# speechbrain/speechbrain

Measured on NVIDIA H100. Metric: audio-sec/sec (RTFx) Conformer-L ASR, batch=32x10s@16kHz, higher is better.
Workload: dtype fp16 operands, fp32 accumulate/residual/softmax

## Files before the change

### speechbrain_b200/csrc/common.cuh

```cuda
#pragma once
#include <cuda.h>
#include <cuda_fp16.h>
#include <cuda_runtime.h>
#include <stdint.h>

#define SBK_OK 0
#define SBK_ERR_CUDA -1
#define SBK_ERR_ARG -2
#define SBK_ERR_UNSUPPORTED -3
#define SBK_ERR_NOMEM -4

namespace sbk {

void set_error(const char* fmt, ...);

#define SBK_CUDA_CHECK(expr)                                                              \
    do {                                                                                  \
        cudaError_t _e = (expr);                                                          \
        if (_e != cudaSuccess) {                                                          \
            sbk::set_error("%s:%d: %s -> %s", __FILE__, __LINE__, #expr, cudaGetErrorString(_e)); \
            return SBK_ERR_CUDA;                                                          \
        }                                                                                 \
    } while (0)

// ... 20 lines not shown
__device__ __forceinline__ void pdl_wait() { asm volatile("griddepcontrol.wait;" ::: "memory"); }

template <typename... KArgs, typename... Args>
inline cudaError_t launch_pdl(void (*kern)(KArgs...), dim3 grid, dim3 block, size_t smem, cudaStream_t st, bool pdl,
                              Args... args) {
    cudaLaunchConfig_t cfg = {};
    cfg.gridDim = grid;
    cfg.blockDim = block;
    cfg.dynamicSmemBytes = smem;
    cfg.stream = st;
    cudaLaunchAttribute attr[1];
    attr[0].id = cudaLaunchAttributeProgrammaticStreamSerialization;
    attr[0].val.programmaticStreamSerializationAllowed = 1;
    cfg.attrs = attr;
    cfg.numAttrs = pdl ? 1 : 0;
    return cudaLaunchKernelEx(&cfg, kern, args...);
}

__device__ __forceinline__ float warp_sum(float v) {
#pragma unroll
    for (int o = 16; o > 0; o >>= 1) v += __shfl_xor_sync(0xffffffffu, v, o);
    return v;
}
__device__ __forceinline__ float warp_max(float v) {
#pragma unroll
    for (int o = 16; o > 0; o >>= 1) v = fmaxf(v, __shfl_xor_sync(0xffffffffu, v, o));
    return v;
}

__device__ __forceinline__ uint32_t smem_u32(const void* p) {
    return static_cast<uint32_t>(__cvta_generic_to_shared(p));
}

__device__ __forceinline__ void mbar_init(uint64_t* bar, uint32_t count) {
    asm volatile("mbarrier.init.shared::cta.b64 [%0], %1;" ::"r"(smem_u32(bar)), "r"(count));
}
__device__ __forceinline__ void mbar_fence_init() {
    asm volatile("fence.mbarrier_init.release.cluster;" ::: "memory");
}
__device__ __forceinline__ void mbar_arrive_expect_tx(uint64_t* bar, uint32_t bytes) {
    asm volatile("mbarrier.arrive.expect_tx.shared::cta.b64 _, [%0], %1;" ::"r"(smem_u32(bar)), "r"(bytes)
                 : "memory");
}
__device__ __forceinline__ void mbar_arrive(uint64_t* bar) {
    asm volatile("mbarrier.arrive.shared::cta.b64 _, [%0];" ::"r"(smem_u32(bar)) : "memory");
}
__device__ __forceinline__ bool mbar_try_wait(uint64_t* bar, uint32_t parity) {
    uint32_t ok;
    asm volatile(
        "{\n\t.reg .pred p;\n\t"
        "mbarrier.try_wait.parity.shared::cta.b64 p, [%1], %2;\n\t"
        "selp.u32 %0, 1, 0, p;\n\t}"
        : "=r"(ok)
        : "r"(smem_u32(bar)), "r"(parity)
        : "memory");
    return ok != 0;
}
__device__ __forceinline__ void mbar_wait(uint64_t* bar, uint32_t parity) {
    while (!mbar_try_wait(bar, parity)) {
    }
}

__device__ __forceinline__ void tma_prefetch_desc(const CUtensorMap* m) {
    asm volatile("prefetch.tensormap [%0];" ::"l"(reinterpret_cast<uint64_t>(m)) : "memory");
}
__device__ __forceinline__ void tma_load_2d(void* smem_dst, const CUtensorMap* m, uint64_t* bar, int c0, int c1) {
    asm volatile(
        "cp.async.bulk.tensor.2d.shared::cluster.global.mbarrier::complete_tx::bytes [%0], [%1, {%3, %4}], [%2];"
        ::"r"(smem_u32(smem_dst)), "l"(reinterpret_cast<uint64_t>(m)), "r"(smem_u32(bar)), "r"(c0), "r"(c1)
        : "memory");
}
__device__ __forceinline__ void tma_load_4d(void* smem_dst, const CUtensorMap* m, uint64_t* bar, int c0, int c1, int c2, int c3) {
    asm volatile(
        "cp.async.bulk.tensor.4d.shared::cluster.global.mbarrier::complete_tx::bytes [%0], [%1, {%3, %4, %5, %6}], [%2];"
        ::"r"(smem_u32(smem_dst)), "l"(reinterpret_cast<uint64_t>(m)), "r"(smem_u32(bar)), "r"(c0), "r"(c1), "r"(c2), "r"(c3)
        : "memory");
}
__device__ __forceinline__ void bulk_load_1d(void* smem_dst, const void* gsrc, uint32_t bytes, uint64_t* bar) {
    asm volatile(
        "cp.async.bulk.shared::cluster.global.mbarrier::complete_tx::bytes [%0], [%1], %2, [%3];"
        ::"r"(smem_u32(smem_dst)), "l"(reinterpret_cast<uint64_t>(gsrc)), "r"(bytes), "r"(smem_u32(bar))
        : "memory");
}

__device__ __forceinline__ void wgmma_fence() { asm volatile("wgmma.fence.sync.aligned;" ::: "memory"); }
__device__ __forceinline__ void wgmma_commit() { asm volatile("wgmma.commit_group.sync.aligned;" ::: "memory"); }
template <int N>
__device__ __forceinline__ void wgmma_wait() { asm volatile("wgmma.wait_group.sync.aligned %0;" ::"n"(N) : "memory"); }

__device__ __forceinline__ uint64_t make_kmajor_sw128_desc(uint32_t smem_addr) {
    uint64_t d = 0;
    d |= static_cast<uint64_t>((smem_addr & 0x3FFFFu) >> 4);
    d |= static_cast<uint64_t>(1) << 16;
    d |= static_cast<uint64_t>(1024 >> 4) << 32;
    d |= static_cast<uint64_t>(1) << 62;
    return d;
}

template <int N>
__device__ __forceinline__ void wgmma_f16(float (&d)[N / 2], uint64_t desc_a, uint64_t desc_b, uint32_t accumulate);
template <>
__device__ __forceinline__ void wgmma_f16<32>(float (&d)[16], uint64_t desc_a, uint64_t desc_b, uint32_t accumulate) {
    asm volatile(
        "{\n\t.reg .pred p;\n\tsetp.ne.b32 p, %18, 0;\n\t"
        "wgmma.mma_async.sync.aligned.m64n32k16.f32.f16.f16 "
        "{%0, %1, %2, %3, %4, %5, %6, %7, %8, %9, %10, %11, %12, %13, %14, %15}, "
        "%16, %17, p, 1, 1, 0, 0;\n\t}"
        : "+f"(d[0]), "+f"(d[1]), "+f"(d[2]), "+f"(d[3]), "+f"(d[4]), "+f"(d[5]), "+f"(d[6]), "+f"(d[7]),
          "+f"(d[8]), "+f"(d[9]), "+f"(d[10]), "+f"(d[11]), "+f"(d[12]), "+f"(d[13]), "+f"(d[14]), "+f"(d[15])
        : "l"(desc_a), "l"(desc_b), "r"(accumulate)
        : "memory");
}
template <>
__device__ __forceinline__ void wgmma_f16<64>(float (&d)[32], uint64_t desc_a, uint64_t desc_b, uint32_t accumulate) {
    asm volatile(
        "{\n\t.reg .pred p;\n\tsetp.ne.b32 p, %34, 0;\n\t"
        "wgmma.mma_async.sync.aligned.m64n64k16.f32.f16.f16 "
        "{%0, %1, %2, %3, %4, %5, %6, %7, %8, %9, %10, %11, %12, %13, %14, %15, "
        "%16, %17, %18, %19, %20, %21, %22, %23, %24, %25, %26, %27, %28, %29, %30, %31}, "
        "%32, %33, p, 1, 1, 0, 0;\n\t}"
        : "+f"(d[0]), "+f"(d[1]), "+f"(d[2]), "+f"(d[3]), "+f"(d[4]), "+f"(d[5]), "+f"(d[6]), "+f"(d[7]),
          "+f"(d[8]), "+f"(d[9]), "+f"(d[10]), "+f"(d[11]), "+f"(d[12]), "+f"(d[13]), "+f"(d[14]), "+f"(d[15]),
          "+f"(d[16]), "+f"(d[17]), "+f"(d[18]), "+f"(d[19]), "+f"(d[20]), "+f"(d[21]), "+f"(d[22]), "+f"(d[23]),
          "+f"(d[24]), "+f"(d[25]), "+f"(d[26]), "+f"(d[27]), "+f"(d[28]), "+f"(d[29]), "+f"(d[30]), "+f"(d[31])
        : "l"(desc_a), "l"(desc_b), "r"(accumulate)
        : "memory");
}
template <>
__device__ __forceinline__ void wgmma_f16<128>(float (&d)[64], uint64_t desc_a, uint64_t desc_b, uint32_t accumulate) {
    asm volatile(
        "{\n\t.reg .pred p;\n\tsetp.ne.b32 p, %66, 0;\n\t"
        "wgmma.mma_async.sync.aligned.m64n128k16.f32.f16.f16 "
        "{%0, %1, %2, %3, %4, %5, %6, %7, %8, %9, %10, %11, %12, %13, %14, %15, "
        "%16, %17, %18, %19, %20, %21, %22, %23, %24, %25, %26, %27, %28, %29, %30, %31, "
        "%32, %33, %34, %35, %36, %37, %38, %39, %40, %41, %42, %43, %44, %45, %46, %47, "
        "%48, %49, %50, %51, %52, %53, %54, %55, %56, %57, %58, %59, %60, %61, %62, %63}, "
        "%64, %65, p, 1, 1, 0, 0;\n\t}"
        : "+f"(d[0]), "+f"(d[1]), "+f"(d[2]), "+f"(d[3]), "+f"(d[4]), "+f"(d[5]), "+f"(d[6]), "+f"(d[7]),
          "+f"(d[8]), "+f"(d[9]), "+f"(d[10]), "+f"(d[11]), "+f"(d[12]), "+f"(d[13]), "+f"(d[14]), "+f"(d[15]),
          "+f"(d[16]), "+f"(d[17]), "+f"(d[18]), "+f"(d[19]), "+f"(d[20]), "+f"(d[21]), "+f"(d[22]), "+f"(d[23]),
          "+f"(d[24]), "+f"(d[25]), "+f"(d[26]), "+f"(d[27]), "+f"(d[28]), "+f"(d[29]), "+f"(d[30]), "+f"(d[31]),
          "+f"(d[32]), "+f"(d[33]), "+f"(d[34]), "+f"(d[35]), "+f"(d[36]), "+f"(d[37]), "+f"(d[38]), "+f"(d[39]),
          "+f"(d[40]), "+f"(d[41]), "+f"(d[42]), "+f"(d[43]), "+f"(d[44]), "+f"(d[45]), "+f"(d[46]), "+f"(d[47]),
          "+f"(d[48]), "+f"(d[49]), "+f"(d[50]), "+f"(d[51]), "+f"(d[52]), "+f"(d[53]), "+f"(d[54]), "+f"(d[55]),
          "+f"(d[56]), "+f"(d[57]), "+f"(d[58]), "+f"(d[59]), "+f"(d[60]), "+f"(d[61]), "+f"(d[62]), "+f"(d[63])
        : "l"(desc_a), "l"(desc_b), "r"(accumulate)
        : "memory");
}

template <>
__device__ __forceinline__ void wgmma_f16<256>(float (&d)[128], uint64_t desc_a, uint64_t desc_b, uint32_t accumulate) {
    asm volatile(
        "{\n\t.reg .pred p;\n\tsetp.ne.b32 p, %130, 0;\n\t"
        "wgmma.mma_async.sync.aligned.m64n256k16.f32.f16.f16 "
        "{"
        "%0, %1, %2, %3, %4, %5, %6, %7, %8, %9, %10, %11, %12, %13, %14, %15, "
        "%16, %17, %18, %19, %20, %21, %22, %23, %24, %25, %26, %27, %28, %29, %30, %31, "
        "%32, %33, %34, %35, %36, %37, %38, %39, %40, %41, %42, %43, %44, %45, %46, %47, "
        "%48, %49, %50, %51, %52, %53, %54, %55, %56, %57, %58, %59, %60, %61, %62, %63, "
        "%64, %65, %66, %67, %68, %69, %70, %71, %72, %73, %74, %75, %76, %77, %78, %79, "
        "%80, %81, %82, %83, %84, %85, %86, %87, %88, %89, %90, %91, %92, %93, %94, %95, "
        "%96, %97, %98, %99, %100, %101, %102, %103, %104, %105, %106, %107, %108, %109, %110, %111, "
        "%112, %113, %114, %115, %116, %117, %118, %119, %120, %121, %122, %123, %124, %125, %126, %127}, "
        "%128, %129, p, 1, 1, 0, 0;\n\t}"
        :
          "+f"(d[0]), "+f"(d[1]), "+f"(d[2]), "+f"(d[3]), "+f"(d[4]), "+f"(d[5]), "+f"(d[6]), "+f"(d[7]),
          "+f"(d[8]), "+f"(d[9]), "+f"(d[10]), "+f"(d[11]), "+f"(d[12]), "+f"(d[13]), "+f"(d[14]), "+f"(d[15]),
          "+f"(d[16]), "+f"(d[17]), "+f"(d[18]), "+f"(d[19]), "+f"(d[20]), "+f"(d[21]), "+f"(d[22]), "+f"(d[23]),
          "+f"(d[24]), "+f"(d[25]), "+f"(d[26]), "+f"(d[27]), "+f"(d[28]), "+f"(d[29]), "+f"(d[30]), "+f"(d[31]),
          "+f"(d[32]), "+f"(d[33]), "+f"(d[34]), "+f"(d[35]), "+f"(d[36]), "+f"(d[37]), "+f"(d[38]), "+f"(d[39]),
          "+f"(d[40]), "+f"(d[41]), "+f"(d[42]), "+f"(d[43]), "+f"(d[44]), "+f"(d[45]), "+f"(d[46]), "+f"(d[47]),
          "+f"(d[48]), "+f"(d[49]), "+f"(d[50]), "+f"(d[51]), "+f"(d[52]), "+f"(d[53]), "+f"(d[54]), "+f"(d[55]),
          "+f"(d[56]), "+f"(d[57]), "+f"(d[58]), "+f"(d[59]), "+f"(d[60]), "+f"(d[61]), "+f"(d[62]), "+f"(d[63]),
          "+f"(d[64]), "+f"(d[65]), "+f"(d[66]), "+f"(d[67]), "+f"(d[68]), "+f"(d[69]), "+f"(d[70]), "+f"(d[71]),
          "+f"(d[72]), "+f"(d[73]), "+f"(d[74]), "+f"(d[75]), "+f"(d[76]), "+f"(d[77]), "+f"(d[78]), "+f"(d[79]),
          "+f"(d[80]), "+f"(d[81]), "+f"(d[82]), "+f"(d[83]), "+f"(d[84]), "+f"(d[85]), "+f"(d[86]), "+f"(d[87]),
          "+f"(d[88]), "+f"(d[89]), "+f"(d[90]), "+f"(d[91]), "+f"(d[92]), "+f"(d[93]), "+f"(d[94]), "+f"(d[95]),
          "+f"(d[96]), "+f"(d[97]), "+f"(d[98]), "+f"(d[99]), "+f"(d[100]), "+f"(d[101]), "+f"(d[102]), "+f"(d[103]),
          "+f"(d[104]), "+f"(d[105]), "+f"(d[106]), "+f"(d[107]), "+f"(d[108]), "+f"(d[109]), "+f"(d[110]), "+f"(d[111]),
          "+f"(d[112]), "+f"(d[113]), "+f"(d[114]), "+f"(d[115]), "+f"(d[116]), "+f"(d[117]), "+f"(d[118]), "+f"(d[119]),
          "+f"(d[120]), "+f"(d[121]), "+f"(d[122]), "+f"(d[123]), "+f"(d[124]), "+f"(d[125]), "+f"(d[126]), "+f"(d[127])
        : "l"(desc_a), "l"(desc_b), "r"(accumulate)
        : "memory");
}

__device__ __forceinline__ __half2 floats2half2_sat(float lo, float hi) {
    uint32_t r;
    asm("cvt.rn.satfinite.f16x2.f32 %0, %1, %2;" : "=r"(r) : "f"(hi), "f"(lo));
    return *reinterpret_cast<__half2*>(&r);
}
__device__ __forceinline__ __half float2half_sat(float x) {
    const __half2 h = floats2half2_sat(x, 0.0f);
    return __low2half(h);
}

__device__ __forceinline__ float rcp_approx(float x) {
    float y;
    asm("rcp.approx.ftz.f32 %0, %1;" : "=f"(y) : "f"(x));
    return y;
}
__device__ __forceinline__ float exp_ftz(float x) {
    float y;
    asm("ex2.approx.ftz.f32 %0, %1;" : "=f"(y) : "f"(x * 1.4426950408889634f));
    return y;
}
__device__ __forceinline__ float sigmoid_f(float x) { return rcp_approx(1.0f + exp_ftz(-x)); }
__device__ __forceinline__ float tanh_approx(float x) {
    float y;
    asm("tanh.approx.f32 %0, %1;" : "=f"(y) : "f"(x));
    return y;
}
__device__ __forceinline__ float sigmoid_fast(float x) { return fmaf(0.5f, tanh_approx(0.5f * x), 0.5f); }
__device__ __forceinline__ float silu_fast(float x) {
    const float h = 0.5f * x;
    return fmaf(h, tanh_approx(h), h);
}
__device__ __forceinline__ void sts128(uint32_t addr, uint4 v) {
    asm volatile("st.shared.v4.b32 [%0], {%1, %2, %3, %4};" ::"r"(addr), "r"(v.x), "r"(v.y), "r"(v.z), "r"(v.w) : "memory");
}
__device__ __forceinline__ uint4 lds128(uint32_t addr) {
    uint4 v;
    asm volatile("ld.shared.v4.b32 {%0, %1, %2, %3}, [%4];" : "=r"(v.x), "=r"(v.y), "=r"(v.z), "=r"(v.w) : "r"(addr) : "memory");
    return v;
}
__device__ __forceinline__ uint4 f4_as_u4(float4 f) {
    return make_uint4(__float_as_uint(f.x), __float_as_uint(f.y), __float_as_uint(f.z), __float_as_uint(f.w));
}
__device__ __forceinline__ float4 u4_as_f4(uint4 u) {
    return make_float4(__uint_as_float(u.x), __uint_as_float(u.y), __uint_as_float(u.z), __uint_as_float(u.w));
}
__device__ __forceinline__ float silu_f(float x) { return x * sigmoid_f(x); }
__device__ __forceinline__ float gelu_erf_f(float x) { return 0.5f * x * (1.0f + erff(x * 0.70710678118654752f)); }

__device__ __forceinline__ int float_to_ordered(float f) {
    int i = __float_as_int(f);
    return i >= 0 ? i : i ^ 0x7FFFFFFF;
}
__device__ __forceinline__ float ordered_to_float(int i) { return __int_as_float(i >= 0 ? i : i ^ 0x7FFFFFFF); }

int make_tmap_2d_f16(CUtensorMap* out, const void* base, uint64_t rows, uint64_t cols, uint64_t row_stride_elems,
                     uint32_t box_rows, uint32_t box_cols);

}
```

### speechbrain_b200/csrc/gemm_tc2.cu

```cuda
#include <stdio.h>
#include <stdlib.h>

#include "common.cuh"
#include "sbk_internal.h"

namespace sbk {

constexpr int PP_BM = 128, PP_BK = 64;
constexpr int PP_THREADS = 384;
constexpr int PP_GROUP_M = 8;
constexpr int PP_A_BYTES = PP_BM * PP_BK * 2;
constexpr int PP_STG_WARP_BYTES = 16 * 160;
constexpr int PP_BAR_TURN = 2;
constexpr int PP_CONSUMER_REGS = 232, PP_PRODUCER_REGS = 40;
static_assert(128 * PP_PRODUCER_REGS + 256 * PP_CONSUMER_REGS <= 65536, "register file");

template <int BN>
struct PpCfg {
    static constexpr bool PINGPONG = BN == 128;
    static constexpr int STAGES = BN == 128 ? 6 : 4;
    static constexpr int STAGE_BYTES = PP_A_BYTES + BN * PP_BK * 2;
    static constexpr int BAR_OFFSET = STAGES * STAGE_BYTES;
    static constexpr int STG_OFFSET = BAR_OFFSET + 128;
    static constexpr int BIAS_OFFSET = STG_OFFSET + 8 * PP_STG_WARP_BYTES;
    static constexpr int SMEM = BIAS_OFFSET + 8 * BN * 4 + 1024;
    static_assert(STAGE_BYTES % 1024 == 0, "128B-swizzled stages must stay 1 KB aligned");
    static_assert(2 * STAGES * 8 <= 128, "mbarriers overflow their slot");
    static_assert(SMEM <= 227 * 1024, "shared memory");
};

template <int MODE>
__host__ __device__ constexpr int pp_stg_pitch() {
    return (MODE == EPI_F32 || MODE == EPI_RESID) ? 160 : MODE == EPI_ROPE ? 144 : 80;
}

__device__ __forceinline__ void named_bar_sync(int id, int n) { asm volatile("bar.sync %0, %1;" ::"r"(id), "r"(n) : "memory"); }
__device__ __forceinline__ void named_bar_arrive(int id, int n) { asm volatile("bar.arrive %0, %1;" ::"r"(id), "r"(n) : "memory"); }
template <int R>
__device__ __forceinline__ void setmaxnreg_inc() { asm volatile("setmaxnreg.inc.sync.aligned.u32 %0;" ::"n"(R)); }
template <int R>
__device__ __forceinline__ void setmaxnreg_dec() { asm volatile("setmaxnreg.dec.sync.aligned.u32 %0;" ::"n"(R)); }
__device__ __forceinline__ void sts32(uint32_t addr, uint32_t v) { asm volatile("st.shared.b32 [%0], %1;" ::"r"(addr), "r"(v) : "memory"); }
__device__ __forceinline__ void sts64(uint32_t addr, float x, float y) {
    asm volatile("st.shared.v2.f32 [%0], {%1, %2};" ::"r"(addr), "f"(x), "f"(y) : "memory");
}
__device__ __forceinline__ float2 lds64(uint32_t addr) {
    float2 v;
    asm volatile("ld.shared.v2.f32 {%0, %1}, [%2];" : "=f"(v.x), "=f"(v.y) : "r"(addr) : "memory");
    return v;
}
__device__ __forceinline__ uint32_t half2_bits(float lo, float hi) {
    const __half2 h = floats2half2_sat(lo, hi);
    return *reinterpret_cast<const uint32_t*>(&h);
}

template <int BN>
__device__ __forceinline__ void pp_tile_coords(int t, int tiles_m, int tiles_n, int& m0, int& n0) {
    const int per_group = PP_GROUP_M * tiles_n;
    const int grp = t / per_group, first_m = grp * PP_GROUP_M;
    const int rows = min(PP_GROUP_M, tiles_m - first_m);
    const int r = t - grp * per_group;
    m0 = (first_m + r % rows) * PP_BM;
    n0 = (r / rows) * BN;
}


template <int MODE>
__device__ __forceinline__ void pp_row_alpha(const GemmEpilogue& e, float (&alpha)[2], int row_base, int M, int lane) {
#pragma unroll
    for (int i = 0; i < 2; ++i) {
        const int row = row_base + (lane >> 2) + 8 * i;
        alpha[i] = e.alpha;
        if (MODE == EPI_RESID && e.row_lens != nullptr && row < M) {
            const int b = row / e.T, t = row - b * e.T;
            if (t >= __ldg(e.row_lens + b)) alpha[i] = 0.0f;
        }
    }
}

__device__ __forceinline__ void pp_resid_prefetch(const GemmEpilogue& e, float4 (&res)[4], int row_base, int col0, int M,
                                                  int lane) {
    const int seg = lane & 7, rsub = lane >> 3;
#pragma unroll
    for (int i = 0; i < 4; ++i) {
        const int row = row_base + i * 4 + rsub;
        res[i] = row < M ? __ldcg(reinterpret_cast<const float4*>(e.resid + static_cast<size_t>(row) * e.ldo + col0 + seg * 4))
                         : make_float4(0.f, 0.f, 0.f, 0.f);
    }
}
__device__ __forceinline__ void pp_rope_prefetch(const GemmEpilogue& e, float4 (&rc)[2], float4 (&rs)[2], int row_base,
                                                 int col0, int lane) {
    const int dh = e.head_dim;
    const int within = col0 % (3 * dh);
    const int sect = within / dh;
    if (sect < 2) {
        const int p = ((within - sect * dh) >> 1) + (lane & 3) * 4;
#pragma unroll
        for (int i = 0; i < 2; ++i) {
            const int t = (row_base + i * 8 + (lane >> 2)) % e.T;
            rc[i] = __ldg(reinterpret_cast<const float4*>(e.rope_cos + static_cast<size_t>(t) * (dh >> 1) + p));
            rs[i] = __ldg(reinterpret_cast<const float4*>(e.rope_sin + static_cast<size_t>(t) * (dh >> 1) + p));
        }
    }
}
template <int MODE>
__device__ __forceinline__ void pp_prefetch(const GemmEpilogue& e, float4 (&res)[4], float4 (&rc)[2], float4 (&rs)[2],
                                            int row_base, int col0, int M, int lane) {
    if constexpr (MODE == EPI_RESID) pp_resid_prefetch(e, res, row_base, col0, M, lane);
    if constexpr (MODE == EPI_ROPE) pp_rope_prefetch(e, rc, rs, row_base, col0, lane);
// ... 59 lines not shown
            if (row < M) {
                float4 val = u4_as_f4(lds128(stg + r * P + seg * 16));
                if constexpr (MODE == EPI_RESID) {
                    val.x += res[i].x; val.y += res[i].y; val.z += res[i].z; val.w += res[i].w;
                }
                *reinterpret_cast<float4*>(outp + static_cast<size_t>(row) * e.ldo + col0 + seg * 4) = val;
            }
        }
    } else if constexpr (MODE == EPI_ROPE) {
        const int seg = lane & 3, rsub = lane >> 2;
        const int dh = e.head_dim;
        const int sect = (col0 % (3 * dh)) / dh;
        const float sc = sect == 0 ? e.alpha : 1.0f;
        __half* outp = reinterpret_cast<__half*>(e.out);
#pragma unroll
        for (int i = 0; i < 2; ++i) {
            const int r = i * 8 + rsub;
            const int row = row_base + r;
            float4 x0 = u4_as_f4(lds128(stg + r * P + seg * 32));
            float4 x1 = u4_as_f4(lds128(stg + r * P + seg * 32 + 16));
            if (sect < 2) {
                const float4 c = rc[i], s4 = rs[i];
                const float a0 = (x0.x * c.x - x0.y * s4.x) * sc, a1 = (x0.y * c.x + x0.x * s4.x) * sc;
                const float a2 = (x0.z * c.y - x0.w * s4.y) * sc, a3 = (x0.w * c.y + x0.z * s4.y) * sc;
                const float b0 = (x1.x * c.z - x1.y * s4.z) * sc, b1 = (x1.y * c.z + x1.x * s4.z) * sc;
                const float b2 = (x1.z * c.w - x1.w * s4.w) * sc, b3 = (x1.w * c.w + x1.z * s4.w) * sc;
                x0 = make_float4(a0, a1, a2, a3);
                x1 = make_float4(b0, b1, b2, b3);
            }
            if (row < M)
                *reinterpret_cast<uint4*>(outp + static_cast<size_t>(row) * e.ldo + col0 + seg * 8) =
                    make_uint4(half2_bits(x0.x, x0.y), half2_bits(x0.z, x0.w), half2_bits(x1.x, x1.y), half2_bits(x1.z, x1.w));
        }
    } else {
        const int seg = lane & 3, rsub = lane >> 2;
        if (MODE == EPI_F16 && e.kv_heads > 0) {
            const int d = e.kv_heads * 64;
            const int layer = col0 / (2 * d), within = col0 - layer * 2 * d;
            const int part = within / d, cc = within - part * d, head = cc >> 6, dcol = cc & 63;
            __half* pbase = reinterpret_cast<__half*>(e.out) + static_cast<size_t>(layer) * e.kv_layer_stride +
                            static_cast<size_t>(part) * e.kv_part_stride;
#pragma unroll
            for (int i = 0; i < 2; ++i) {
                const int r = i * 8 + rsub;
                const int row = row_base + r;
                if (row < M) {
                    const int b = row / e.T, t = row - b * e.T;
                    __half* dst = pbase + ((static_cast<size_t>(b) * e.kv_heads + head) * e.T + t) * 64 + dcol + seg * 8;
                    *reinterpret_cast<uint4*>(dst) = lds128(stg + r * P + seg * 16);
                }
            }
        } else {
            uint8_t* outp = reinterpret_cast<uint8_t*>(e.out);
            const size_t row_pitch = MODE == EPI_GLU ? static_cast<size_t>(e.ldo) * 4 : static_cast<size_t>(e.ldo) * 2;
            const size_t col_off = static_cast<size_t>(col0) * 2;
#pragma unroll
            for (int i = 0; i < 2; ++i) {
                const int r = i * 8 + rsub;
                const int row = row_base + r;
                if (row < M)
                    *reinterpret_cast<uint4*>(outp + static_cast<size_t>(row) * row_pitch + col_off + seg * 16) =
                        lds128(stg + r * P + seg * 16);
            }
        }
    }
    __syncwarp();
}

template <int MODE, int ACT>
__device__ __forceinline__ void pp_epilogue_rows(const GemmEpilogue& e, const float (&a)[64], uint32_t stg, uint32_t sbias,
                                                 const float (&alpha)[2], int row_base, int n0, int M, int lane,
                                                 float4 (&res)[4], float4 (&rc)[2], float4 (&rs)[2], bool has_next,
                                                 int next_row_base, int next_n0) {
    pp_epilogue_chunk<MODE, ACT, 0>(e, a, stg, sbias, alpha, row_base, n0, M, lane, res, rc, rs);
    pp_prefetch<MODE>(e, res, rc, rs, row_base, n0 + 32, M, lane);
    pp_epilogue_chunk<MODE, ACT, 1>(e, a, stg, sbias, alpha, row_base, n0 + 32, M, lane, res, rc, rs);
    pp_prefetch<MODE>(e, res, rc, rs, row_base, n0 + 64, M, lane);
    pp_epilogue_chunk<MODE, ACT, 2>(e, a, stg, sbias, alpha, row_base, n0 + 64, M, lane, res, rc, rs);
    pp_prefetch<MODE>(e, res, rc, rs, row_base, n0 + 96, M, lane);
    pp_epilogue_chunk<MODE, ACT, 3>(e, a, stg, sbias, alpha, row_base, n0 + 96, M, lane, res, rc, rs);
    if (has_next) pp_prefetch<MODE>(e, res, rc, rs, next_row_base, next_n0, M, lane);
}

template <int MODE, int ACT, int BN>
__global__ void __launch_bounds__(PP_THREADS, 1)
gemm_tc2_kernel(const __grid_constant__ CUtensorMap tmap_a, const __grid_constant__ CUtensorMap tmap_b,
                const GemmEpilogue epi, int M, int N, int K) {
    using C = PpCfg<BN>;
    constexpr int ST = C::STAGES;
    extern __shared__ uint8_t smem_raw[];
    uint8_t* smem = reinterpret_cast<uint8_t*>((reinterpret_cast<uintptr_t>(smem_raw) + 1023) & ~uintptr_t(1023));
    uint64_t* full_bar = reinterpret_cast<uint64_t*>(smem + C::BAR_OFFSET);
    uint64_t* empty_bar = full_bar + ST;
    const int num_kb = (K + PP_BK - 1) / PP_BK;
    const int tiles_m = (M + PP_BM - 1) / PP_BM, tiles_n = N / BN, tiles = tiles_m * tiles_n;

    if (threadIdx.x == 0) {
        tma_prefetch_desc(&tmap_a);
        tma_prefetch_desc(&tmap_b);
        for (int s = 0; s < ST; ++s) {
            mbar_init(&full_bar[s], 1);
            mbar_init(&empty_bar[s], C::PINGPONG ? 1 : 2);
        }
        mbar_fence_init();
    }
    __syncthreads();
    const int wg = threadIdx.x >> 7;
    if (wg == 0) {
        setmaxnreg_dec<PP_PRODUCER_REGS>();
        if (threadIdx.x == 0) {
            int it = 0;
            for (int t = blockIdx.x; t < tiles; t += gridDim.x) {
                int m0, n0;
                pp_tile_coords<BN>(t, tiles_m, tiles_n, m0, n0);
                for (int kb = 0; kb < num_kb; ++kb, ++it) {
                    const int s = it % ST;
                    mbar_wait(&empty_bar[s], ((it / ST) & 1) ^ 1);
                    mbar_arrive_expect_tx(&full_bar[s], C::STAGE_BYTES);
                    uint8_t* dst = smem + s * C::STAGE_BYTES;
                    tma_load_2d(dst, &tmap_a, &full_bar[s], kb * PP_BK, m0);
                    tma_load_2d(dst + PP_A_BYTES, &tmap_b, &full_bar[s], kb * PP_BK, n0);
                }
            }
        }
        return;
    }
    setmaxnreg_inc<PP_CONSUMER_REGS>();
    const int g = wg - 1;
    const int warp = (threadIdx.x >> 5) & 3, lane = threadIdx.x & 31;
    const uint32_t stg = smem_u32(smem + C::STG_OFFSET + (g * 4 + warp) * PP_STG_WARP_BYTES);
    const uint32_t sbias = smem_u32(smem + C::BIAS_OFFSET + (g * 4 + warp) * BN * 4);
    constexpr int STEP = C::PINGPONG ? 2 : 1;
    int j = C::PINGPONG ? g : 0;
    for (int t = blockIdx.x + (C::PINGPONG ? g : 0) * gridDim.x; t < tiles; t += STEP * gridDim.x, j += STEP) {
        int m0, n0;
        pp_tile_coords<BN>(t, tiles_m, tiles_n, m0, n0);
        const int rb0 = m0 + (C::PINGPONG ? 0 : 64 * g) + warp * 16, rb1 = C::PINGPONG ? rb0 + 64 : rb0;
        const int cb1 = C::PINGPONG ? n0 : n0 + 128;
        float4 res[4], rc[2], rs[2];
        pp_prefetch<MODE>(epi, res, rc, rs, rb0, n0, M, lane);
        float4 bias4[BN / 128];
#pragma unroll
        for (int q = 0; q < BN / 128; ++q)
            bias4[q] = epi.bias != nullptr ? __ldg(reinterpret_cast<const float4*>(epi.bias + n0 + 128 * q) + lane)
                                           : make_float4(0.f, 0.f, 0.f, 0.f);
        float alpha[2][2];
        if constexpr (MODE == EPI_RESID) {
            pp_row_alpha<MODE>(epi, alpha[0], rb0, M, lane);
            pp_row_alpha<MODE>(epi, alpha[1], rb1, M, lane);
        }
        float acc[2][64];
#pragma unroll
        for (int h = 0; h < 2; ++h)
#pragma unroll
            for (int x = 0; x < 64; ++x) acc[h][x] = 0.0f;
        if (C::PINGPONG && j > 0) named_bar_sync(PP_BAR_TURN + g, 256);
        int it = j * num_kb;
        for (int kb = 0; kb < num_kb; ++kb, ++it) {
            const int s = it % ST;
            mbar_wait(&full_bar[s], (it / ST) & 1);
            const uint32_t a_addr = smem_u32(smem + s * C::STAGE_BYTES);
            const uint64_t db = make_kmajor_sw128_desc(a_addr + PP_A_BYTES);
            wgmma_fence();
#pragma unroll
            for (int k = 0; k < PP_BK / 16; ++k) {
                if constexpr (C::PINGPONG) {
#pragma unroll
                    for (int h = 0; h < 2; ++h)
                        wgmma_f16<128>(acc[h], make_kmajor_sw128_desc(a_addr + h * 64 * 128) + 2 * k, db + 2 * k, 1u);
                } else {
                    wgmma_f16<256>(reinterpret_cast<float(&)[128]>(acc), make_kmajor_sw128_desc(a_addr + g * 64 * 128) + 2 * k,
                                   db + 2 * k, 1u);
                }
            }
            wgmma_commit();
            wgmma_wait<1>();
            if (kb > 0 && (threadIdx.x & 127) == 0) mbar_arrive(&empty_bar[(it - 1) % ST]);
        }
        if (C::PINGPONG && t + gridDim.x < tiles) named_bar_arrive(PP_BAR_TURN + (g ^ 1), 256);
        wgmma_wait<0>();
        if ((threadIdx.x & 127) == 0) mbar_arrive(&empty_bar[(it - 1) % ST]);
#pragma unroll
        for (int q = 0; q < BN / 128; ++q)
            sts128(sbias + q * 512 + lane * 16, f4_as_u4(bias4[q]));
        __syncwarp();
        pp_epilogue_rows<MODE, ACT>(epi, acc[0], stg, sbias, alpha[0], rb0, n0, M, lane, res, rc, rs, true, rb1, cb1);
        pp_epilogue_rows<MODE, ACT>(epi, acc[1], stg, sbias + (cb1 - n0) * 4, alpha[1], rb1, cb1, M, lane, res, rc, rs, false,
                                    0, 0);
    }
}

using WideKernel = void (*)(const CUtensorMap, const CUtensorMap, const GemmEpilogue, int, int, int);
template <int BN>
static WideKernel pick_wide_kernel(const GemmEpilogue& epi, bool fast_act) {
    switch (epi.mode) {
        case EPI_F16:
            if (epi.act == ACT_SILU) return fast_act ? gemm_tc2_kernel<EPI_F16, ACT_SILU_FAST, BN> : gemm_tc2_kernel<EPI_F16, ACT_SILU, BN>;
            if (epi.act == ACT_GELU) return gemm_tc2_kernel<EPI_F16, ACT_GELU, BN>;
            if (epi.act == ACT_NONE) return gemm_tc2_kernel<EPI_F16, ACT_NONE, BN>;
            return nullptr;
        case EPI_F32: return gemm_tc2_kernel<EPI_F32, ACT_NONE, BN>;
        case EPI_RESID: return gemm_tc2_kernel<EPI_RESID, ACT_NONE, BN>;
        case EPI_GLU: return fast_act ? gemm_tc2_kernel<EPI_GLU, ACT_SILU_FAST, BN> : gemm_tc2_kernel<EPI_GLU, ACT_NONE, BN>;
        case EPI_ROPE: return gemm_tc2_kernel<EPI_ROPE, ACT_NONE, BN>;
        default: return nullptr;
    }
}

int gemm_f16_wide(const void* A, int lda, const void* W, int ldw, const GemmEpilogue& epi, int M, int N, int K,
                  cudaStream_t stream) {
    const int bn = (epi.mode == EPI_F32 || epi.mode == EPI_RESID) && K <= 1024 ? 128 : 256;
    CUtensorMap ta, tb;
    int rc = make_tmap_2d_f16(&ta, A, M, K, lda, PP_BM, PP_BK);
    if (rc) return rc;
    rc = make_tmap_2d_f16(&tb, W, N, K, ldw, bn, PP_BK);
    if (rc) return rc;
    static const bool fast_act = getenv("SBK_SILU_EXACT") == nullptr;
    const WideKernel kern = bn == 128 ? pick_wide_kernel<128>(epi, fast_act) : pick_wide_kernel<256>(epi, fast_act);
    if (kern == nullptr) { set_error("gemm_f16_wide: epilogue mode %d / activation %d not built", epi.mode, epi.act); return SBK_ERR_ARG; }
    const int smem = bn == 128 ? PpCfg<128>::SMEM : PpCfg<256>::SMEM;
    SBK_CUDA_CHECK(cudaFuncSetAttribute(kern, cudaFuncAttributeMaxDynamicSharedMemorySize, smem));
    int dev = 0, sms = 0;
    SBK_CUDA_CHECK(cudaGetDevice(&dev));
    SBK_CUDA_CHECK(cudaDeviceGetAttribute(&sms, cudaDevAttrMultiProcessorCount, dev));
    const int tiles = ceil_div(M, PP_BM) * (N / bn);
    const int rounds = ceil_div(tiles, sms);
    const int grid = ceil_div(tiles, rounds);
    GemmProfile* prof = gemm_profile();
    cudaEvent_t e0 = nullptr, e1 = nullptr;
    if (prof->enabled) {
        cudaEventCreate(&e0);
        cudaEventCreate(&e1);
        cudaEventRecord(e0, stream);
    }
    kern<<<grid, PP_THREADS, smem, stream>>>(ta, tb, epi, M, N, K);
    if (prof->enabled) {
        cudaEventRecord(e1, stream);
        prof->ev.push_back(e0);
        prof->ev.push_back(e1);
        prof->flops.push_back(2.0 * M * N * K);
        prof->shape.insert(prof->shape.end(), {M, N, K, epi.mode});
    }
    SBK_LAUNCH_CHECK();
    return SBK_OK;
}

}
```

### speechbrain_b200/csrc/tma_host.cu

```cuda
#include <cudaTypedefs.h>
#include <stdarg.h>
#include <stdio.h>

#include "common.cuh"
#include "sbk_internal.h"

namespace sbk {

static thread_local char g_err[1024] = "";

void set_error(const char* fmt, ...) {
    va_list ap;
    va_start(ap, fmt);
    vsnprintf(g_err, sizeof(g_err), fmt, ap);
    va_end(ap);
}
const char* last_error() { return g_err; }

static long long g_launches = 0;
static bool g_capturing = false;
static long long g_capture_count = 0;
void count_launch() {
    if (g_capturing) ++g_capture_count;
    else ++g_launches;
}
void launch_count_begin_capture() { g_capturing = true; g_capture_count = 0; }
long long launch_count_end_capture() { g_capturing = false; return g_capture_count; }
void launch_count_add(long long n) { g_launches += n; }
long long launch_count() { return g_launches; }

static GemmProfile g_prof;
GemmProfile* gemm_profile() { return &g_prof; }

static PFN_cuTensorMapEncodeTiled_v12000 get_encode_fn() {
    static PFN_cuTensorMapEncodeTiled_v12000 fn = nullptr;
    if (fn) return fn;
    void* p = nullptr;
    cudaDriverEntryPointQueryResult q;
    if (cudaGetDriverEntryPoint("cuTensorMapEncodeTiled", &p, cudaEnableDefault, &q) != cudaSuccess ||
        q != cudaDriverEntryPointSuccess)
        return nullptr;
    fn = reinterpret_cast<PFN_cuTensorMapEncodeTiled_v12000>(p);
    return fn;
}

int make_tmap_2d_f16(CUtensorMap* out, const void* base, uint64_t rows, uint64_t cols, uint64_t row_stride_elems,
                     uint32_t box_rows, uint32_t box_cols) {
    auto fn = get_encode_fn();
    if (!fn) {
        set_error("cuTensorMapEncodeTiled driver entry point unavailable (no CUDA driver?)");
        return SBK_ERR_CUDA;
    }
    cuuint64_t gdim[2] = {cols, rows};
    cuuint64_t gstride[1] = {row_stride_elems * 2};
    cuuint32_t box[2] = {box_cols, box_rows};
    cuuint32_t estr[2] = {1, 1};
    CUresult r = fn(out, CU_TENSOR_MAP_DATA_TYPE_FLOAT16, 2, const_cast<void*>(base), gdim, gstride, box, estr,
                    CU_TENSOR_MAP_INTERLEAVE_NONE, CU_TENSOR_MAP_SWIZZLE_128B, CU_TENSOR_MAP_L2_PROMOTION_L2_256B,
                    CU_TENSOR_MAP_FLOAT_OOB_FILL_NONE);
    if (r != CUDA_SUCCESS) {
        set_error("cuTensorMapEncodeTiled failed (%d) rows=%llu cols=%llu stride=%llu", (int)r,
                  (unsigned long long)rows, (unsigned long long)cols, (unsigned long long)row_stride_elems);
        return SBK_ERR_CUDA;
    }
    return SBK_OK;
}


int make_tmap_kv_f16(CUtensorMap* out, const void* base, int n_utt, int T, int H, uint64_t key_stride_elems,
                     uint64_t utt_stride_elems, int box_T) {
    auto fn = get_encode_fn();
    if (!fn) {
        set_error("cuTensorMapEncodeTiled driver entry point unavailable (no CUDA driver?)");
        return SBK_ERR_CUDA;
    }
    cuuint64_t gdim[4] = {64, static_cast<cuuint64_t>(2 * H), static_cast<cuuint64_t>(T), static_cast<cuuint64_t>(n_utt)};
    cuuint64_t gstride[3] = {128, key_stride_elems * 2, utt_stride_elems * 2};
    cuuint32_t box[4] = {64, 1, static_cast<cuuint32_t>(box_T), 1};
    cuuint32_t estr[4] = {1, 1, 1, 1};
    CUresult r = fn(out, CU_TENSOR_MAP_DATA_TYPE_FLOAT16, 4, const_cast<void*>(base), gdim, gstride, box, estr,
                    CU_TENSOR_MAP_INTERLEAVE_NONE, CU_TENSOR_MAP_SWIZZLE_NONE, CU_TENSOR_MAP_L2_PROMOTION_L2_128B,
                    CU_TENSOR_MAP_FLOAT_OOB_FILL_NONE);
    if (r != CUDA_SUCCESS) {
        set_error("cuTensorMapEncodeTiled(kv) failed (%d) n_utt=%d T=%d H=%d", (int)r, n_utt, T, H);
        return SBK_ERR_CUDA;
    }
    return SBK_OK;
}

int make_tmap_2d_f32(CUtensorMap* out, const void* base, uint64_t rows, uint64_t cols, uint32_t box_cols) {
    auto fn = get_encode_fn();
    if (!fn) {
        set_error("cuTensorMapEncodeTiled driver entry point unavailable (no CUDA driver?)");
        return SBK_ERR_CUDA;
    }
    cuuint64_t gdim[2] = {cols, rows};
    cuuint64_t gstride[1] = {cols * 4};
    cuuint32_t box[2] = {box_cols, 1};
    cuuint32_t estr[2] = {1, 1};
    CUresult r = fn(out, CU_TENSOR_MAP_DATA_TYPE_FLOAT32, 2, const_cast<void*>(base), gdim, gstride, box, estr,
                    CU_TENSOR_MAP_INTERLEAVE_NONE, CU_TENSOR_MAP_SWIZZLE_NONE, CU_TENSOR_MAP_L2_PROMOTION_L2_128B,
                    CU_TENSOR_MAP_FLOAT_OOB_FILL_NONE);
    if (r != CUDA_SUCCESS) {
        set_error("cuTensorMapEncodeTiled(f32) failed (%d)", (int)r);
        return SBK_ERR_CUDA;
    }
    return SBK_OK;
}

}
```

Measured before the change: 44230.

## Add TMA-store epilogue for wide BN=256 GEMM f16 and GLU outputs

New measurement: 44360, median of 6. Within noise of the previous version (+0.3%).

```diff
diff --git a/speechbrain_b200/csrc/common.cuh b/speechbrain_b200/csrc/common.cuh
--- a/speechbrain_b200/csrc/common.cuh
+++ b/speechbrain_b200/csrc/common.cuh
@@ -126,6 +126,22 @@
         ::"r"(smem_u32(smem_dst)), "l"(reinterpret_cast<uint64_t>(gsrc)), "r"(bytes), "r"(smem_u32(bar))
         : "memory");
 }
+
+__device__ __forceinline__ void tma_store_2d(const CUtensorMap* m, uint32_t smem_src, int c0, int c1) {
+    asm volatile("cp.async.bulk.tensor.2d.global.shared::cta.bulk_group [%0, {%2, %3}], [%1];"
+                 ::"l"(reinterpret_cast<uint64_t>(m)), "r"(smem_src), "r"(c0), "r"(c1)
+                 : "memory");
+}
+__device__ __forceinline__ void tma_store_3d(const CUtensorMap* m, uint32_t smem_src, int c0, int c1, int c2) {
+    asm volatile("cp.async.bulk.tensor.3d.global.shared::cta.bulk_group [%0, {%2, %3, %4}], [%1];"
+                 ::"l"(reinterpret_cast<uint64_t>(m)), "r"(smem_src), "r"(c0), "r"(c1), "r"(c2)
+                 : "memory");
+}
+__device__ __forceinline__ void tma_store_commit() { asm volatile("cp.async.bulk.commit_group;" ::: "memory"); }
+template <int N>
+__device__ __forceinline__ void tma_store_wait_read() { asm volatile("cp.async.bulk.wait_group.read %0;" ::"n"(N) : "memory"); }
+__device__ __forceinline__ void tma_store_wait_all() { asm volatile("cp.async.bulk.wait_group 0;" ::: "memory"); }
+__device__ __forceinline__ void fence_proxy_async_smem() { asm volatile("fence.proxy.async.shared::cta;" ::: "memory"); }
 
 __device__ __forceinline__ void wgmma_fence() { asm volatile("wgmma.fence.sync.aligned;" ::: "memory"); }
 __device__ __forceinline__ void wgmma_commit() { asm volatile("wgmma.commit_group.sync.aligned;" ::: "memory"); }
@@ -284,5 +300,8 @@
 
 int make_tmap_2d_f16(CUtensorMap* out, const void* base, uint64_t rows, uint64_t cols, uint64_t row_stride_elems,
                      uint32_t box_rows, uint32_t box_cols);
-
-}
+int make_tmap_2d_sw128(CUtensorMap* out, const void* base, int elem_bytes, uint64_t rows, uint64_t cols,
+                       uint64_t row_stride_elems, uint32_t box_rows, uint32_t box_cols);
+int make_tmap_kv_scatter(CUtensorMap* out, const void* base, int panels, int T);
+
+}
diff --git a/speechbrain_b200/csrc/gemm_tc2.cu b/speechbrain_b200/csrc/gemm_tc2.cu
--- a/speechbrain_b200/csrc/gemm_tc2.cu
+++ b/speechbrain_b200/csrc/gemm_tc2.cu
@@ -14,17 +14,23 @@
 constexpr int PP_BAR_TURN = 2;
 constexpr int PP_CONSUMER_REGS = 232, PP_PRODUCER_REGS = 40;
 static_assert(128 * PP_PRODUCER_REGS + 256 * PP_CONSUMER_REGS <= 65536, "register file");
+constexpr int PP_OUT_SLOTS = 2, PP_OUT_SLOT_BYTES = 64 * 128;
+constexpr int PP_BAR_EPI = 4;
+static_assert(4 % PP_OUT_SLOTS == 0 && PP_OUT_SLOTS >= 2, "a tile's four quarters cycle through the slots");
 
 template <int BN>
 struct PpCfg {
     static constexpr bool PINGPONG = BN == 128;
     static constexpr int STAGES = BN == 128 ? 6 : 4;
     static constexpr int STAGE_BYTES = PP_A_BYTES + BN * PP_BK * 2;
-    static constexpr int BAR_OFFSET = STAGES * STAGE_BYTES;
-    static constexpr int STG_OFFSET = BAR_OFFSET + 128;
+    static constexpr int EPI_OFFSET = STAGES * STAGE_BYTES;
+    static constexpr int STG_OFFSET = EPI_OFFSET;
     static constexpr int BIAS_OFFSET = STG_OFFSET + 8 * PP_STG_WARP_BYTES;
-    static constexpr int SMEM = BIAS_OFFSET + 8 * BN * 4 + 1024;
-    static_assert(STAGE_BYTES % 1024 == 0, "128B-swizzled stages must stay 1 KB aligned");
+    static constexpr int REG_EPI_BYTES = 8 * PP_STG_WARP_BYTES + 8 * BN * 4;
+    static constexpr int TMA_EPI_BYTES = PINGPONG ? 0 : 2 * PP_OUT_SLOTS * PP_OUT_SLOT_BYTES;
+    static constexpr int BAR_OFFSET = EPI_OFFSET + (REG_EPI_BYTES > TMA_EPI_BYTES ? REG_EPI_BYTES : TMA_EPI_BYTES);
+    static constexpr int SMEM = BAR_OFFSET + 128 + 1024;
+    static_assert(STAGE_BYTES % 1024 == 0, "128B-swizzled stages and output slots must stay 1 KB aligned");
     static_assert(2 * STAGES * 8 <= 128, "mbarriers overflow their slot");
     static_assert(SMEM <= 227 * 1024, "shared memory");
 };
@@ -250,11 +256,94 @@
     if (has_next) pp_prefetch<MODE>(e, res, rc, rs, next_row_base, next_n0, M, lane);
 }
 
-template <int MODE, int ACT, int BN>
+
+template <int MODE, int ACT, int CH>
+__device__ __forceinline__ void pp_tma_chunk(const GemmEpilogue& e, const float (&a)[128], uint32_t srow, int col0, int lane) {
+    const int qc = 2 * (lane & 3), r0 = lane >> 2;
+    float v[4][2][2];
+#pragma unroll
+    for (int q = 0; q < 4; ++q) {
+        const float2 b = e.bias != nullptr ? __ldg(reinterpret_cast<const float2*>(e.bias + col0 + 8 * q + qc))
+                                           : make_float2(0.f, 0.f);
+#pragma unroll
+        for (int i = 0; i < 2; ++i) {
+            v[q][i][0] = a[4 * (4 * CH + q) + 2 * i] + b.x;
+            v[q][i][1] = a[4 * (4 * CH + q) + 2 * i + 1] + b.y;
+        }
+    }
+    if constexpr (MODE == EPI_GLU) {
+#pragma unroll
+        for (int q = 0; q < 2; ++q)
+#pragma unroll
+            for (int i = 0; i < 2; ++i) {
+                float o[2];
+#pragma unroll
+                for (int c = 0; c < 2; ++c)
+                    o[c] = ACT == ACT_SILU_FAST ? v[q][i][c] * sigmoid_fast(v[q + 2][i][c]) : v[q][i][c] * sigmoid_f(v[q + 2][i][c]);
+                sts64(srow + 1024 * i + (((4 * (CH & 1) + 2 * q + (qc >> 2)) ^ r0) << 4) + 4 * (qc & 3), o[0], o[1]);
+            }
+    } else {
+#pragma unroll
+        for (int q = 0; q < 4; ++q)
+#pragma unroll
+            for (int i = 0; i < 2; ++i) {
+#pragma unroll
+                for (int c = 0; c < 2; ++c) {
+                    if constexpr (ACT == ACT_SILU) v[q][i][c] = silu_f(v[q][i][c]);
+                    else if constexpr (ACT == ACT_SILU_FAST) v[q][i][c] = silu_fast(v[q][i][c]);
+                    else if constexpr (ACT == ACT_GELU) v[q][i][c] = gelu_erf_f(v[q][i][c]);
+                }
+                sts32(srow + 1024 * i + (((4 * (CH & 1) + q) ^ r0) << 4) + 2 * qc, half2_bits(v[q][i][0], v[q][i][1]));
+            }
+    }
+}
+
+template <int MODE, int ACT, int QT>
+__device__ __forceinline__ void pp_tma_quarter(const CUtensorMap* tmap_o, const GemmEpilogue& e, const float (&a)[128],
+                                               uint32_t slots, int g, int warp, int lane, int m0, int n0, int M) {
+    const uint32_t slot = slots + (QT % PP_OUT_SLOTS) * PP_OUT_SLOT_BYTES;
+    const uint32_t srow = slot + (16 * warp + (lane >> 2)) * 128;
+    const int col0 = n0 + 64 * QT;
+    pp_tma_chunk<MODE, ACT, 2 * QT>(e, a, srow, col0, lane);
+    pp_tma_chunk<MODE, ACT, 2 * QT + 1>(e, a, srow, col0 + 32, lane);
+    fence_proxy_async_smem();
+    const bool leader = (threadIdx.x & 127) == 0;
+    if (leader) tma_store_wait_read<PP_OUT_SLOTS - 2>();
+    named_bar_sync(PP_BAR_EPI + g, 128);
+    if (MODE == EPI_F16 && e.kv_heads > 0) {
+        const int d = e.kv_heads * 64, lp = col0 / d, head = (col0 - lp * d) >> 6;
+        const int r = m0 + 64 * g, b = r / e.T, t0 = r - b * e.T;
+        const int n_utt = M / e.T;
+        if (t0 + 64 <= e.T) {
+            if (leader && r < M) {
+                tma_store_3d(tmap_o, slot, 0, t0, (lp * n_utt + b) * e.kv_heads + head);
+                tma_store_commit();
+            }
+        } else {
+#pragma unroll
+            for (int k = 0; k < 4; ++k) {
+                const int c = (threadIdx.x & 127) + 128 * k, R = c >> 3, x = c & 7;
+                const int row = r + R;
+                if (row < M) {
+                    const int bb = row / e.T, t = row - bb * e.T;
+                    __half* dst = reinterpret_cast<__half*>(e.out) + static_cast<size_t>(lp) * e.kv_part_stride +
+                                  ((static_cast<size_t>(bb) * e.kv_heads + head) * e.T + t) * 64 + x * 8;
+                    *reinterpret_cast<uint4*>(dst) = lds128(slot + R * 128 + ((x ^ (R & 7)) << 4));
+                }
+            }
+        }
+    } else if (leader) {
+        tma_store_2d(tmap_o, slot, MODE == EPI_GLU ? col0 / 2 : col0, m0 + 64 * g);
+        tma_store_commit();
+    }
+}
+
+template <int MODE, int ACT, int BN, bool TMA_EPI>
 __global__ void __launch_bounds__(PP_THREADS, 1)
 gemm_tc2_kernel(const __grid_constant__ CUtensorMap tmap_a, const __grid_constant__ CUtensorMap tmap_b,
-                const GemmEpilogue epi, int M, int N, int K) {
+                const __grid_constant__ CUtensorMap tmap_o, const GemmEpilogue epi, int M, int N, int K) {
     using C = PpCfg<BN>;
+    static_assert(!TMA_EPI || (BN == 256 && (MODE == EPI_F16 || MODE == EPI_GLU)), "TMA-store epilogue");
     constexpr int ST = C::STAGES;
     extern __shared__ uint8_t smem_raw[];
     uint8_t* smem = reinterpret_cast<uint8_t*>((reinterpret_cast<uintptr_t>(smem_raw) + 1023) & ~uintptr_t(1023));
@@ -266,6 +355,7 @@
     if (threadIdx.x == 0) {
         tma_prefetch_desc(&tmap_a);
         tma_prefetch_desc(&tmap_b);
+        if constexpr (TMA_EPI) tma_prefetch_desc(&tmap_o);
         for (int s = 0; s < ST; ++s) {
             mbar_init(&full_bar[s], 1);
             mbar_init(&empty_bar[s], C::PINGPONG ? 1 : 2);
@@ -298,6 +388,7 @@
     const int warp = (threadIdx.x >> 5) & 3, lane = threadIdx.x & 31;
     const uint32_t stg = smem_u32(smem + C::STG_OFFSET + (g * 4 + warp) * PP_STG_WARP_BYTES);
     const uint32_t sbias = smem_u32(smem + C::BIAS_OFFSET + (g * 4 + warp) * BN * 4);
+    const uint32_t slots = smem_u32(smem + C::EPI_OFFSET + g * PP_OUT_SLOTS * PP_OUT_SLOT_BYTES);
     constexpr int STEP = C::PINGPONG ? 2 : 1;
     int j = C::PINGPONG ? g : 0;
     for (int t = blockIdx.x + (C::PINGPONG ? g : 0) * gridDim.x; t < tiles; t += STEP * gridDim.x, j += STEP) {
@@ -306,12 +397,14 @@
         const int rb0 = m0 + (C::PINGPONG ? 0 : 64 * g) + warp * 16, rb1 = C::PINGPONG ? rb0 + 64 : rb0;
         const int cb1 = C::PINGPONG ? n0 : n0 + 128;
         float4 res[4], rc[2], rs[2];
-        pp_prefetch<MODE>(epi, res, rc, rs, rb0, n0, M, lane);
         float4 bias4[BN / 128];
-#pragma unroll
-        for (int q = 0; q < BN / 128; ++q)
-            bias4[q] = epi.bias != nullptr ? __ldg(reinterpret_cast<const float4*>(epi.bias + n0 + 128 * q) + lane)
-                                           : make_float4(0.f, 0.f, 0.f, 0.f);
+        if constexpr (!TMA_EPI) {
+            pp_prefetch<MODE>(epi, res, rc, rs, rb0, n0, M, lane);
+#pragma unroll
+            for (int q = 0; q < BN / 128; ++q)
+                bias4[q] = epi.bias != nullptr ? __ldg(reinterpret_cast<const float4*>(epi.bias + n0 + 128 * q) + lane)
+                                               : make_float4(0.f, 0.f, 0.f, 0.f);
+        }
         float alpha[2][2];
         if constexpr (MODE == EPI_RESID) {
             pp_row_alpha<MODE>(epi, alpha[0], rb0, M, lane);
@@ -348,29 +441,53 @@
         if (C::PINGPONG && t + gridDim.x < tiles) named_bar_arrive(PP_BAR_TURN + (g ^ 1), 256);
         wgmma_wait<0>();
         if ((threadIdx.x & 127) == 0) mbar_arrive(&empty_bar[(it - 1) % ST]);
-#pragma unroll
-        for (int q = 0; q < BN / 128; ++q)
-            sts128(sbias + q * 512 + lane * 16, f4_as_u4(bias4[q]));
-        __syncwarp();
-        pp_epilogue_rows<MODE, ACT>(epi, acc[0], stg, sbias, alpha[0], rb0, n0, M, lane, res, rc, rs, true, rb1, cb1);
-        pp_epilogue_rows<MODE, ACT>(epi, acc[1], stg, sbias + (cb1 - n0) * 4, alpha[1], rb1, cb1, M, lane, res, rc, rs, false,
-                                    0, 0);
-    }
-}
-
-using WideKernel = void (*)(const CUtensorMap, const CUtensorMap, const GemmEpilogue, int, int, int);
+        if constexpr (TMA_EPI) {
+            const float(&a)[128] = reinterpret_cast<const float(&)[128]>(acc);
+            pp_tma_quarter<MODE, ACT, 0>(&tmap_o, epi, a, slots, g, warp, lane, m0, n0, M);
+            pp_tma_quarter<MODE, ACT, 1>(&tmap_o, epi, a, slots, g, warp, lane, m0, n0, M);
+            pp_tma_quarter<MODE, ACT, 2>(&tmap_o, epi, a, slots, g, warp, lane, m0, n0, M);
+            pp_tma_quarter<MODE, ACT, 3>(&tmap_o, epi, a, slots, g, warp, lane, m0, n0, M);
+        } else {
+#pragma unroll
+            for (int q = 0; q < BN / 128; ++q)
+                sts128(sbias + q * 512 + lane * 16, f4_as_u4(bias4[q]));
+            __syncwarp();
+            pp_epilogue_rows<MODE, ACT>(epi, acc[0], stg, sbias, alpha[0], rb0, n0, M, lane, res, rc, rs, true, rb1, cb1);
+            pp_epilogue_rows<MODE, ACT>(epi, acc[1], stg, sbias + (cb1 - n0) * 4, alpha[1], rb1, cb1, M, lane, res, rc, rs,
+                                        false, 0, 0);
+        }
+    }
+    if constexpr (TMA_EPI) {
+        if ((threadIdx.x & 127) == 0) tma_store_wait_all();
+    }
+}
+
+using WideKernel = void (*)(const CUtensorMap, const CUtensorMap, const CUtensorMap, const GemmEpilogue, int, int, int);
 template <int BN>
 static WideKernel pick_wide_kernel(const GemmEpilogue& epi, bool fast_act) {
     switch (epi.mode) {
         case EPI_F16:
-            if (epi.act == ACT_SILU) return fast_act ? gemm_tc2_kernel<EPI_F16, ACT_SILU_FAST, BN> : gemm_tc2_kernel<EPI_F16, ACT_SILU, BN>;
-            if (epi.act == ACT_GELU) return gemm_tc2_kernel<EPI_F16, ACT_GELU, BN>;
-            if (epi.act == ACT_NONE) return gemm_tc2_kernel<EPI_F16, ACT_NONE, BN>;
+            if (epi.act == ACT_SILU)
+                return fast_act ? gemm_tc2_kernel<EPI_F16, ACT_SILU_FAST, BN, false> : gemm_tc2_kernel<EPI_F16, ACT_SILU, BN, false>;
+            if (epi.act == ACT_GELU) return gemm_tc2_kernel<EPI_F16, ACT_GELU, BN, false>;
+            if (epi.act == ACT_NONE) return gemm_tc2_kernel<EPI_F16, ACT_NONE, BN, false>;
             return nullptr;
-        case EPI_F32: return gemm_tc2_kernel<EPI_F32, ACT_NONE, BN>;
-        case EPI_RESID: return gemm_tc2_kernel<EPI_RESID, ACT_NONE, BN>;
-        case EPI_GLU: return fast_act ? gemm_tc2_kernel<EPI_GLU, ACT_SILU_FAST, BN> : gemm_tc2_kernel<EPI_GLU, ACT_NONE, BN>;
-        case EPI_ROPE: return gemm_tc2_kernel<EPI_ROPE, ACT_NONE, BN>;
+        case EPI_F32: return gemm_tc2_kernel<EPI_F32, ACT_NONE, BN, false>;
+        case EPI_RESID: return gemm_tc2_kernel<EPI_RESID, ACT_NONE, BN, false>;
+        case EPI_GLU: return fast_act ? gemm_tc2_kernel<EPI_GLU, ACT_SILU_FAST, BN, false> : gemm_tc2_kernel<EPI_GLU, ACT_NONE, BN, false>;
+        case EPI_ROPE: return gemm_tc2_kernel<EPI_ROPE, ACT_NONE, BN, false>;
+        default: return nullptr;
+    }
+}
+static WideKernel pick_wide_tma_kernel(const GemmEpilogue& epi, bool fast_act) {
+    switch (epi.mode) {
+        case EPI_F16:
+            if (epi.act == ACT_SILU)
+                return fast_act ? gemm_tc2_kernel<EPI_F16, ACT_SILU_FAST, 256, true> : gemm_tc2_kernel<EPI_F16, ACT_SILU, 256, true>;
+            if (epi.act == ACT_GELU) return gemm_tc2_kernel<EPI_F16, ACT_GELU, 256, true>;
+            if (epi.act == ACT_NONE) return gemm_tc2_kernel<EPI_F16, ACT_NONE, 256, true>;
+            return nullptr;
+        case EPI_GLU: return fast_act ? gemm_tc2_kernel<EPI_GLU, ACT_SILU_FAST, 256, true> : gemm_tc2_kernel<EPI_GLU, ACT_NONE, 256, true>;
         default: return nullptr;
     }
 }
@@ -378,13 +495,32 @@
 int gemm_f16_wide(const void* A, int lda, const void* W, int ldw, const GemmEpilogue& epi, int M, int N, int K,
                   cudaStream_t stream) {
     const int bn = (epi.mode == EPI_F32 || epi.mode == EPI_RESID) && K <= 1024 ? 128 : 256;
-    CUtensorMap ta, tb;
+    CUtensorMap ta, tb, to;
     int rc = make_tmap_2d_f16(&ta, A, M, K, lda, PP_BM, PP_BK);
     if (rc) return rc;
     rc = make_tmap_2d_f16(&tb, W, N, K, ldw, bn, PP_BK);
     if (rc) return rc;
+    const int out_bytes = epi.mode == EPI_GLU ? 4 : 2;
+    const bool kv_scatter = epi.mode == EPI_F16 && epi.kv_heads > 0;
+    const int kv_d = epi.kv_heads * 64;
+    const bool tma_epi =
+        bn == 256 && getenv("SBK_GEMM_REG_EPI") == nullptr && (epi.mode == EPI_GLU || epi.mode == EPI_F16) &&
+        reinterpret_cast<uintptr_t>(epi.out) % 16 == 0 &&
+        (kv_scatter ? epi.T >= 64 && M % epi.T == 0 && epi.kv_part_stride == static_cast<size_t>(M) * kv_d &&
+                          (N == 2 * kv_d || epi.kv_layer_stride == 2 * epi.kv_part_stride)
+                    : (static_cast<size_t>(epi.ldo) * out_bytes) % 16 == 0);
+    if (tma_epi && kv_scatter) {
+        rc = make_tmap_kv_scatter(&to, epi.out, N / kv_d * (M / epi.T) * epi.kv_heads, epi.T);
+        if (rc) return rc;
+    } else if (tma_epi) {
+        rc = make_tmap_2d_sw128(&to, epi.out, out_bytes, M, epi.mode == EPI_GLU ? N / 2 : N, epi.ldo, 64, 128 / out_bytes);
+        if (rc) return rc;
+    } else {
+        to = tb;
+    }
     static const bool fast_act = getenv("SBK_SILU_EXACT") == nullptr;
-    const WideKernel kern = bn == 128 ? pick_wide_kernel<128>(epi, fast_act) : pick_wide_kernel<256>(epi, fast_act);
+    const WideKernel kern = tma_epi ? pick_wide_tma_kernel(epi, fast_act)
+                            : bn == 128 ? pick_wide_kernel<128>(epi, fast_act) : pick_wide_kernel<256>(epi, fast_act);
     if (kern == nullptr) { set_error("gemm_f16_wide: epilogue mode %d / activation %d not built", epi.mode, epi.act); return SBK_ERR_ARG; }
     const int smem = bn == 128 ? PpCfg<128>::SMEM : PpCfg<256>::SMEM;
     SBK_CUDA_CHECK(cudaFuncSetAttribute(kern, cudaFuncAttributeMaxDynamicSharedMemorySize, smem));
@@ -401,7 +537,7 @@
         cudaEventCreate(&e1);
         cudaEventRecord(e0, stream);
     }
-    kern<<<grid, PP_THREADS, smem, stream>>>(ta, tb, epi, M, N, K);
+    kern<<<grid, PP_THREADS, smem, stream>>>(ta, tb, to, epi, M, N, K);
     if (prof->enabled) {
         cudaEventRecord(e1, stream);
         prof->ev.push_back(e0);
diff --git a/speechbrain_b200/csrc/tma_host.cu b/speechbrain_b200/csrc/tma_host.cu
--- a/speechbrain_b200/csrc/tma_host.cu
+++ b/speechbrain_b200/csrc/tma_host.cu
@@ -66,6 +66,47 @@
     return SBK_OK;
 }
 
+int make_tmap_2d_sw128(CUtensorMap* out, const void* base, int elem_bytes, uint64_t rows, uint64_t cols,
+                       uint64_t row_stride_elems, uint32_t box_rows, uint32_t box_cols) {
+    auto fn = get_encode_fn();
+    if (!fn) {
+        set_error("cuTensorMapEncodeTiled driver entry point unavailable (no CUDA driver?)");
+        return SBK_ERR_CUDA;
+    }
+    cuuint64_t gdim[2] = {cols, rows};
+    cuuint64_t gstride[1] = {row_stride_elems * elem_bytes};
+    cuuint32_t box[2] = {box_cols, box_rows};
+    cuuint32_t estr[2] = {1, 1};
+    CUresult r = fn(out, elem_bytes == 4 ? CU_TENSOR_MAP_DATA_TYPE_FLOAT32 : CU_TENSOR_MAP_DATA_TYPE_FLOAT16, 2,
+                    const_cast<void*>(base), gdim, gstride, box, estr, CU_TENSOR_MAP_INTERLEAVE_NONE,
+                    CU_TENSOR_MAP_SWIZZLE_128B, CU_TENSOR_MAP_L2_PROMOTION_NONE, CU_TENSOR_MAP_FLOAT_OOB_FILL_NONE);
+    if (r != CUDA_SUCCESS) {
+        set_error("cuTensorMapEncodeTiled(sw128) failed (%d) rows=%llu cols=%llu stride=%llu", (int)r,
+                  (unsigned long long)rows, (unsigned long long)cols, (unsigned long long)row_stride_elems);
+        return SBK_ERR_CUDA;
+    }
+    return SBK_OK;
+}
+
+int make_tmap_kv_scatter(CUtensorMap* out, const void* base, int panels, int T) {
+    auto fn = get_encode_fn();
+    if (!fn) {
+        set_error("cuTensorMapEncodeTiled driver entry point unavailable (no CUDA driver?)");
+        return SBK_ERR_CUDA;
+    }
+    cuuint64_t gdim[3] = {64, static_cast<cuuint64_t>(T), static_cast<cuuint64_t>(panels)};
+    cuuint64_t gstride[2] = {128, static_cast<cuuint64_t>(T) * 128};
+    cuuint32_t box[3] = {64, 64, 1};
+    cuuint32_t estr[3] = {1, 1, 1};
+    CUresult r = fn(out, CU_TENSOR_MAP_DATA_TYPE_FLOAT16, 3, const_cast<void*>(base), gdim, gstride, box, estr,
+                    CU_TENSOR_MAP_INTERLEAVE_NONE, CU_TENSOR_MAP_SWIZZLE_128B, CU_TENSOR_MAP_L2_PROMOTION_NONE,
+                    CU_TENSOR_MAP_FLOAT_OOB_FILL_NONE);
+    if (r != CUDA_SUCCESS) {
+        set_error("cuTensorMapEncodeTiled(kv scatter) failed (%d) panels=%d T=%d", (int)r, panels, T);
+        return SBK_ERR_CUDA;
+    }
+    return SBK_OK;
+}
 
 int make_tmap_kv_f16(CUtensorMap* out, const void* base, int n_utt, int T, int H, uint64_t key_stride_elems,
                      uint64_t utt_stride_elems, int box_T) {
```
